# timmeinhardt/trackformer

Measured on AMD Instinct MI355X. Metric: frames/sec, TrackFormer-Deformable inference (ResNet-50, 1333x800, 300 object + 100 track queries, bs 1 per GPU); roofline = ms_deform_attn HBM GB/s, higher is better.
Workload: dtype f32 (dense layers as the fp16 split product on MFMA: two fp16 pieces per activation, three per weight scaled per output channel -- 22 + 1 significand bits per operand, the one dropped product < 2^-22 --, three terms, f32 accumulate)

## Files before the change

include/tf_fused.h:

```cpp
#ifndef TF_FUSED_H_
#define TF_FUSED_H_

#include <stdint.h>

#ifdef __cplusplus
extern "C" {
#endif

int tf_bias_act_f32(float *x, const float *bias, const float *residual, int64_t n, int C, int relu,
                    void *stream);

int tf_add_layernorm_f32(const float *x, const float *res, const float *gamma, const float *beta,
                         float *out, int64_t rows, int C, float eps, void *stream);

int tf_box_refine_f32(const float *delta, const float *ref, float *out, int64_t rows, int ref_dim, float eps, void *stream);

int tf_postprocess_pack_f32(const float *logits, const float *boxes, float *out, int64_t Q, int C, float img_h, float img_w,
                            int clip, void *stream);

int tf_groupnorm_nhwc_f32(const float *x, const float *gamma, const float *beta, float *out, double *workspace, int N,
                          int HW, int C, int G, float eps, int64_t x_image_stride, int64_t out_image_stride, void *stream);
int tf_groupnorm_stats_nhwc_f32(const float *x, double *workspace, int N, int HW, int C, int G, int64_t x_image_stride, void *stream);
int tf_groupnorm_relu_nhwc_f32(const float *x, const float *gamma, const float *beta, float *out, double *workspace, int N,
                               int HW, int C, int G, float eps, int64_t x_image_stride, int64_t out_image_stride, void *stream);
// ... 76 lines not shown
                         void *stream);

int tf_conv_packed_f32(const float *x, const void *w_packed, const float *bias, const float *residual, float *y, float *workspace,
                       int ksplit, int nimg, int hin, int win, int cin, int cout, int ks, int stride, int relu, int terms,
                       void *stream);

int tf_linear_res_ln_f32(const float *x, const void *w_packed, const float *bias, const float *residual, const float *ln_weight,
                         const float *ln_bias, float ln_eps, float *y, int64_t M, int K, int N, int terms, void *stream);

int tf_ffn_fused_f32(const float *x, const void *w1_packed, const float *b1, const void *w2_packed, const float *b2,
                     const float *residual, const float *ln_weight, const float *ln_bias, float ln_eps, float *y, int64_t M,
                     int d_model, int d_ffn, int terms, void *stream);

typedef struct tf_proj_group {
    const void *w_packed;
    const float *bias;
    float *y;
    int N;
    int add_x2;
} tf_proj_group;
int tf_linear_groups_f32(const float *x, const float *x2, const tf_proj_group *groups, int ngroups, int64_t M, int K, int terms,
                         void *stream);

int tf_mha_core_f32(const float *q, const float *k, const float *v, float *out, const unsigned char *key_mask,
                    int N, int Lq, int Lk, int H, int D, int ldq, int ldk, int ldv, int ldo, float scale,
                    void *stream);

int tf_nms_host_f32(const float *boxes, const float *scores, int n, float iou_threshold, int64_t *keep, int *n_keep);

#ifdef __cplusplus
}
#endif
#endif
```

include/tf_msda.h:

```cpp
#ifndef TF_MSDA_H_
#define TF_MSDA_H_

#include <stdint.h>

#ifdef __cplusplus
extern "C" {
#endif

#define TF_MSDA_ABI_VERSION 9
#define TF_MSDA_MAX_LEVELS 16

typedef enum tf_msda_status {
    TF_MSDA_OK = 0,
    TF_MSDA_ERR_NULL_POINTER = -1,
    TF_MSDA_ERR_BAD_DIMS = -2,
    TF_MSDA_ERR_SHAPE_SUM = -3,
    TF_MSDA_ERR_LAUNCH = -4,
    TF_MSDA_ERR_NO_DEVICE = -5,
    TF_MSDA_ERR_WORKSPACE = -6
} tf_msda_status;

int tf_msda_abi_version(void);

const char *tf_msda_strerror(int status);

int tf_msda_last_hip_error(void);

const char *tf_msda_last_kernel(void);

int tf_msda_set_tiled(int mode);

int tf_msda_set_option(const char *name, int value);
// ... 79 lines not shown
```

trackformer_amd/_cabi.py:

```python
import ctypes
import os

_PKG_DIR = os.path.dirname(os.path.abspath(__file__))
LIB_PATH = os.environ.get("TF_MSDA_LIB") or os.path.join(_PKG_DIR, "lib", "libtf_msda.so")

EXPORTED_SYMBOLS = (
    "tf_msda_abi_version",
    "tf_msda_strerror",
    "tf_msda_last_hip_error",
    "tf_msda_last_kernel",
    "tf_msda_set_tiled",
    "tf_msda_set_option",
    "tf_msda_debug_trace_buffer",
    "tf_msda_forward_fused_f32",
    "tf_msda_forward_f32",
    "tf_msda_forward_f64",
    "tf_msda_forward_f32_dshapes",
    "tf_msda_forward_f64_dshapes",
    "tf_msda_backward_f32",
    "tf_msda_backward_f64",
    "tf_msda_backward_f32_dshapes",
    "tf_msda_backward_f64_dshapes",
    "tf_msda_backward_det_workspace_bytes",
    "tf_msda_backward_det_f32",
# ... 26 lines not shown
    "tf_conv1x1_strided_split_f32",
    "tf_conv1x1_splitk_f32",
    "tf_linear_packed_bytes",
    "tf_linear_pack_weight_f32",
    "tf_linear_packed_f32",
    "tf_linear_grad_stats_workspace_bytes",
    "tf_linear_grad_stats_f32",
    "tf_linear_wgrad_workspace_bytes",
    "tf_linear_wgrad_split_f32",
    "tf_linear_dgrad_packed_f32",
    "tf_add_layernorm_train_f32",
    "tf_add_layernorm_bwd_workspace_bytes",
    "tf_add_layernorm_bwd_f32",
    "tf_set_criterion_fwd_f32",
    "tf_set_criterion_bwd_f32",
    "tf_match_cost_f32",
    "tf_mask_loss_workspace_bytes",
    "tf_mask_loss_fwd_f32",
    "tf_mask_loss_bwd_f32",
    "tf_linear_split_add_f32",
    "tf_ffn_fused_f32",
    "tf_linear_res_ln_f32",
    "tf_linear_groups_f32",
    "tf_conv_packed_f32",
    "tf_mha_core_f32",
    "tf_nms_host_f32",
)

ABI_VERSION = 9

_lib = None


class ProjGroup(ctypes.Structure):
    _fields_ = [("w_packed", ctypes.c_void_p), ("bias", ctypes.c_void_p), ("y", ctypes.c_void_p), ("N", ctypes.c_int),
                ("add_x2", ctypes.c_int)]


class MSDAError(RuntimeError):
    """Raised when libtf_msda.so reports a non-zero status."""


def lib():
    global _lib
    if _lib is not None:
        return _lib
    if not os.path.exists(LIB_PATH):
        raise RuntimeError(
            "trackformer_amd: native library %s not found. Build it with "
            "`python -m trackformer_amd.build` (needs hipcc); there is no CPU fallback." % LIB_PATH)
    import torch
    L = ctypes.CDLL(LIB_PATH)
# ... 67 lines not shown
        fn.argtypes = [vp, vp, vp, vp, vp, ci, ci, ci, ci, ctypes.c_float, ctypes.c_int64, ctypes.c_int64, vp]
    L.tf_linear_split_f32.restype = ci
    L.tf_linear_split_f32.argtypes = [vp, vp, vp, vp, vp, vp, vp, ctypes.c_int64, ci, ci, ci, vp]
    L.tf_linear_split_res_f32.restype = ci
    L.tf_linear_split_res_f32.argtypes = [vp, vp, vp, vp, vp, vp, vp, vp, ctypes.c_int64, ci, ci, ci, vp]
    L.tf_conv3x3_splitk_f32.restype = ci
    L.tf_conv3x3_splitk_f32.argtypes = [vp, vp, vp, vp, vp, vp, vp, vp, ci, ci, ci, ci, ci, ci, ci, ci, vp]
    L.tf_conv3x3_split_f32.restype = ci
    L.tf_conv3x3_split_f32.argtypes = [vp, vp, vp, vp, vp, vp, vp] + [ci] * 7 + [vp]
    L.tf_conv1x1_splitk_f32.restype = ci
    L.tf_conv1x1_splitk_f32.argtypes = [vp, vp, vp, vp, vp, vp, vp, vp, ci, ci, ci, ci, ci, ci, ci, ci, vp]
    L.tf_conv1x1_strided_split_f32.restype = ci
    L.tf_conv1x1_strided_split_f32.argtypes = [vp, vp, vp, vp, vp, vp, vp] + [ci] * 7 + [vp]
    L.tf_linear_packed_bytes.restype = ctypes.c_int64
    L.tf_linear_packed_bytes.argtypes = [ci, ci, ci]
    L.tf_linear_pack_weight_f32.restype = ci
    L.tf_linear_pack_weight_f32.argtypes = [vp, vp, ci, ci, ci, vp]
    L.tf_linear_res_ln_f32.restype = ci
    L.tf_linear_res_ln_f32.argtypes = [vp, vp, vp, vp, vp, vp, ctypes.c_float, vp, ctypes.c_int64, ci, ci, ci, vp]
    L.tf_ffn_fused_f32.restype = ci
    L.tf_ffn_fused_f32.argtypes = [vp, vp, vp, vp, vp, vp, vp, vp, ctypes.c_float, vp, ctypes.c_int64, ci, ci, ci, vp]
    L.tf_linear_groups_f32.restype = ci
    L.tf_linear_groups_f32.argtypes = [vp, vp, ctypes.POINTER(ProjGroup), ci, ctypes.c_int64, ci, ci, vp]
    L.tf_linear_split_add_f32.restype = ci
    L.tf_linear_split_add_f32.argtypes = [vp, vp, vp, vp, vp, vp, vp, vp, ctypes.c_int64, ci, ci, vp]
    L.tf_linear_packed_f32.restype = ci
    L.tf_linear_packed_f32.argtypes = [vp, vp, vp, vp, vp, ctypes.c_int64, ci, ci, ci, ci, vp]
    i64 = ctypes.c_int64
    L.tf_linear_grad_stats_workspace_bytes.restype = i64
    L.tf_linear_grad_stats_workspace_bytes.argtypes = [i64, ci, ci, ci]
    L.tf_linear_grad_stats_f32.restype = ci
    L.tf_linear_grad_stats_f32.argtypes = [vp, vp, vp, vp, i64, i64, ci, ci, ci, vp]
    L.tf_linear_wgrad_workspace_bytes.restype = i64
    L.tf_linear_wgrad_workspace_bytes.argtypes = [i64, ci, ci]
    L.tf_linear_wgrad_split_f32.restype = ci
    L.tf_linear_wgrad_split_f32.argtypes = [vp, vp, vp, vp, vp, vp, i64, i64, ci, ci, ci, vp]
    L.tf_linear_dgrad_packed_f32.restype = ci
    L.tf_linear_dgrad_packed_f32.argtypes = [vp, vp, vp, vp, i64, ci, ci, ci, vp]
    L.tf_add_layernorm_train_f32.restype = ci
    L.tf_add_layernorm_train_f32.argtypes = [vp, vp, vp, vp, vp, vp, i64, ci, ctypes.c_float, vp]
    L.tf_add_layernorm_bwd_workspace_bytes.restype = i64
    L.tf_add_layernorm_bwd_workspace_bytes.argtypes = [i64, ci]
    L.tf_add_layernorm_bwd_f32.restype = ci
    L.tf_add_layernorm_bwd_f32.argtypes = [vp] * 9 + [i64, i64, ci, vp]
    cf = ctypes.c_float
    L.tf_set_criterion_fwd_f32.restype = ci
# ... 29 lines not shown
```

trackformer_amd/backbone.py:

```python
from collections import OrderedDict
from typing import Dict, List

import torch
import torch.nn.functional as F
from torch import nn

from . import fused
from .nested import NestedTensor, all_valid_mask, is_all_valid
from .position_encoding import build_position_encoding


import os as _os

CHANNELS_LAST = _os.environ.get("TF_BACKBONE_NCHW", "0") != "1"


_conv1x1_split = _os.environ.get("TF_CONV1X1_SPLIT", "1") != "0"


_conv3x3_split = _os.environ.get("TF_CONV3X3_SPLIT", "1") != "0"


def _parse_skip(text):
    out = set()
# ... 259 lines not shown
            and maxpool.padding == 1 and maxpool.dilation == 1 and not maxpool.ceil_mode):
        return None
    b = cache.get(conv1, bn1)
    w = cache.weight
    y = None
    if (conv1.kernel_size == (7, 7) and conv1.stride == (2, 2) and conv1.padding == (3, 3) and conv1.dilation == (1, 1)
            and conv1.groups == 1):
        fuse_pool = fused.stem_pool_fused_enabled()
        y = fused.stem_conv(x, w, None if fuse_pool else b, relu=not fuse_pool)
        if y is not None and not fuse_pool:
            return maxpool(y)
    if y is None:
        if not fused.stem_pool_fused_enabled():
            return None
        y = F.conv2d(x, w, None, conv1.stride, conv1.padding, conv1.dilation, conv1.groups)
    pooled = fused.bias_relu_maxpool(y, b)
    if pooled is None:
        if fused.bias_act_(y, b, None, True) is None:
            y = F.relu_(y + b.reshape(1, -1, 1, 1))
        pooled = maxpool(y)
    return pooled


class Bottleneck(nn.Module):
    expansion = 4

    def __init__(self, inplanes, planes, stride=1, downsample=None, dilation=1,
                 norm_layer=FrozenBatchNorm2d):
        super().__init__()
        self.conv1 = nn.Conv2d(inplanes, planes, kernel_size=1, bias=False)
        self.bn1 = norm_layer(planes)
        self.conv2 = nn.Conv2d(planes, planes, kernel_size=3, stride=stride, padding=dilation,
                               dilation=dilation, bias=False)
        self.bn2 = norm_layer(planes)
        self.conv3 = nn.Conv2d(planes, planes * self.expansion, kernel_size=1, bias=False)
        self.bn3 = norm_layer(planes * self.expansion)
        self.relu = nn.ReLU(inplace=True)
        self.downsample = downsample
        self.stride = stride
        self._folds = [_FoldCache() for _ in range(4)]

    def forward(self, x):
        fold = _fold_mode(self, x)
        out = _conv_bn(x, self.conv1, self.bn1, self._folds[0], True, fold)
        out = _conv_bn(out, self.conv2, self.bn2, self._folds[1], True, fold)
        if self.downsample is not None:
            x = _conv_bn(x, self.downsample[0], self.downsample[1], self._folds[3], False, fold)
        return _conv_bn(out, self.conv3, self.bn3, self._folds[2], True, fold, residual=x)


class ResNet(nn.Module):

    def __init__(self, layers, num_classes=1000, replace_stride_with_dilation=None,
                 norm_layer=FrozenBatchNorm2d):
        super().__init__()
        if replace_stride_with_dilation is None:
            replace_stride_with_dilation = [False, False, False]
        if len(replace_stride_with_dilation) != 3:
            raise ValueError("replace_stride_with_dilation should be None or a 3-element tuple")
        self._norm_layer = norm_layer
        self.inplanes = 64
        self.dilation = 1
        self.conv1 = nn.Conv2d(3, 64, kernel_size=7, stride=2, padding=3, bias=False)
        self.bn1 = norm_layer(64)
        self.relu = nn.ReLU(inplace=True)
        self.maxpool = nn.MaxPool2d(kernel_size=3, stride=2, padding=1)
        self.layer1 = self._make_layer(64, layers[0])
        self.layer2 = self._make_layer(128, layers[1], 2, replace_stride_with_dilation[0])
        self.layer3 = self._make_layer(256, layers[2], 2, replace_stride_with_dilation[1])
        self.layer4 = self._make_layer(512, layers[3], 2, replace_stride_with_dilation[2])
        self.avgpool = nn.AdaptiveAvgPool2d((1, 1))
# ... 16 lines not shown
        if stride != 1 or self.inplanes != planes * Bottleneck.expansion:
            downsample = nn.Sequential(
                nn.Conv2d(self.inplanes, planes * Bottleneck.expansion, kernel_size=1, stride=stride,
                          bias=False),
                norm_layer(planes * Bottleneck.expansion))
        layers = [Bottleneck(self.inplanes, planes, stride, downsample, previous_dilation, norm_layer)]
        self.inplanes = planes * Bottleneck.expansion
        for _ in range(1, blocks):
            layers.append(Bottleneck(self.inplanes, planes, dilation=self.dilation,
                                     norm_layer=norm_layer))
        return nn.Sequential(*layers)

    def stem(self, x):
        fold = _fold_mode(self.conv1, x) if self.training else int(_inference_mode(self))
        if fold == 1:
            pooled = _stem_pooled(x, self.conv1, self.bn1, self.maxpool, self._stem_fold)
            if pooled is not None:
                return pooled
        x = _conv_bn(x, self.conv1, self.bn1, self._stem_fold, True, fold)
        return self.maxpool(x)

    def forward(self, x):
        x = self.stem(x)
        x = self.layer4(self.layer3(self.layer2(self.layer1(x))))
        return self.fc(torch.flatten(self.avgpool(x), 1))


_RESNET_DEPTHS = {"resnet50": [3, 4, 6, 3], "resnet101": [3, 4, 23, 3]}


def resnet(name: str, replace_stride_with_dilation=None, norm_layer=FrozenBatchNorm2d) -> ResNet:
    if name not in _RESNET_DEPTHS:
        raise ValueError("unsupported backbone %r (have %s)" % (name, sorted(_RESNET_DEPTHS)))
    return ResNet(_RESNET_DEPTHS[name], replace_stride_with_dilation=replace_stride_with_dilation,
                  norm_layer=norm_layer)


class IntermediateLayerGetter(nn.ModuleDict):

    def __init__(self, model: nn.Module, return_layers: Dict[str, str]):
        if not set(return_layers).issubset(name for name, _ in model.named_children()):
            raise ValueError("return_layers are not present in model")
        remaining = dict(return_layers)
        kept = OrderedDict()
        for name, module in model.named_children():
            kept[name] = module
            remaining.pop(name, None)
            if not remaining:
                break
        super().__init__(kept)
        self.return_layers = dict(return_layers)
        self._fold = _FoldCache()

    def forward(self, x):
        out = OrderedDict()
        fold = _fold_mode(self["conv1"], x) if (self.training and "conv1" in self) else int(_inference_mode(self))
        fused_stem = fold == 1 and all(k in self for k in ("conv1", "bn1", "relu"))
        pooled_stem = (fused_stem and "maxpool" in self
                       and not any(k in self.return_layers for k in ("conv1", "bn1", "relu", "maxpool")))
        skip = ()
        for name, module in self.items():
            if name in skip or (fused_stem and name in ("bn1", "relu")):
                continue
            if fused_stem and name == "conv1":
                pooled = _stem_pooled(x, self["conv1"], self["bn1"], self["maxpool"], self._fold) if pooled_stem else None
                if pooled is not None:
                    x, skip = pooled, ("maxpool",)
                    continue
                x = _conv_bn(x, self["conv1"], self["bn1"], self._fold, True, 1)
            else:
                x = module(x)
            if name in self.return_layers:
                out[self.return_layers[name]] = x
        return out


class BackboneBase(nn.Module):
    def __init__(self, backbone: nn.Module, train_backbone: bool, return_interm_layers: bool):
        super().__init__()
        for name, parameter in backbone.named_parameters():
            if not train_backbone or not any(k in name for k in ("layer2", "layer3", "layer4")):
                parameter.requires_grad_(False)
        if return_interm_layers:
            return_layers = {"layer1": "0", "layer2": "1", "layer3": "2", "layer4": "3"}
            self.strides = [4, 8, 16, 32]
# ... 58 lines not shown
```

trackformer_amd/build.py:

```python
import hashlib
import os
import shutil
import subprocess
import sys
from concurrent.futures import ThreadPoolExecutor

PKG_DIR = os.path.dirname(os.path.abspath(__file__))
REPO_DIR = os.path.dirname(PKG_DIR)
CSRC = os.path.join(PKG_DIR, "csrc")
LIB_DIR = os.path.join(PKG_DIR, "lib")
INCLUDE = os.path.join(REPO_DIR, "include")
GFX_ARCH = "gfx950"

_TARGETS = [
    ("libtf_msda.so", ["msda_hip.hip", "msda_pquad.hip", "fused_ops.hip", "linear_split.hip", "linear_stream.hip", "mha_core.hip", "ffn_fused.hip", "stem_conv.hip", "msda_host.cpp"], []),
]


def _hipcc():
    exe = shutil.which("hipcc") or "/opt/rocm/bin/hipcc"
    if not os.path.exists(exe):
        raise RuntimeError("hipcc not found (expected on PATH or at /opt/rocm/bin/hipcc)")
    return exe

# ... 37 lines not shown
        src_paths = [os.path.join(CSRC, s) for s in srcs]
        flags = ["--offload-arch=" + GFX_ARCH, "-O3", "-std=c++17", "-fPIC", "-I" + INCLUDE,
                 "-Wno-pass-failed"] + extra
        key = _key(src_paths + headers, flags)
        if not force and not _stale(out, key):
            continue
        obj_dir = os.path.join(LIB_DIR, "obj")
        os.makedirs(obj_dir, exist_ok=True)
        objs = [os.path.join(obj_dir, os.path.splitext(s)[0] + ".o") for s in srcs]
        with ThreadPoolExecutor(max_workers=len(srcs)) as pool:
            list(pool.map(lambda so: _run([_hipcc()] + flags + ["-c", so[0], "-o", so[1]], verbose),
                          zip(src_paths, objs)))
        _run([_hipcc(), "--offload-arch=" + GFX_ARCH, "-shared", "-fPIC", "-pthread"] + objs + ["-o", out], verbose)
        _stamp(out, key)
        built.append(out)
    built += _build_tools(force, verbose)
    return built


def _build_tools(force, verbose):
    out_dir = os.path.join(REPO_DIR, "tools", "bin")
    lib = os.path.join(LIB_DIR, "libtf_msda.so")
    built = []
    for name in ("msda_bench", "linear_bench", "ffn_bench", "proj_groups_bench"):
        src = os.path.join(REPO_DIR, "tools", name + ".cpp")
        if not os.path.exists(src):
            continue
        os.makedirs(out_dir, exist_ok=True)
        out = os.path.join(out_dir, name)
        flags = ["--offload-arch=" + GFX_ARCH, "-O2", "-std=c++17", "-I" + INCLUDE]
        headers = [os.path.join(INCLUDE, f) for f in os.listdir(INCLUDE) if f.endswith(".h")]
        key = _key([src] + headers, flags)
        if not force and not _stale(out, key) and os.path.getmtime(out) >= os.path.getmtime(lib):
            continue
        _run([_hipcc()] + flags + [src, "-L" + LIB_DIR, "-ltf_msda",
                                   "-Wl,-rpath,$ORIGIN/../../trackformer_amd/lib", "-o", out], verbose)
        _stamp(out, key)
        built.append(out)
    return built


if __name__ == "__main__":
    res = build_all(force="--force" in sys.argv, verbose=True)
    print("built:" if res else "up to date", *res)
```

trackformer_amd/csrc/ffn_fused.hip:

```cpp
#include <hip/hip_runtime.h>

#include <stdint.h>
#include <stdlib.h>

#include <type_traits>

#include "host_dispatch.h"
#include "msda_common.h"
#include "split_product.h"
#include "tf_fused.h"
#include "tf_msda.h"

namespace {

template <int D>
struct Geo {
    static_assert(D == 256 || D == 288, "hidden sizes of the reference's configurations");
    static constexpr int NW = D == 256 ? 4 : 3;
    static constexpr int NT = NW * 64;
    static constexpr int TJ = D / 32 / NW;
    static constexpr int XS = D + 8;
    static constexpr int CH = NW * 32;
    static constexpr int HS = CH + 8;
    static constexpr int KQ1 = D / 16;
// ... 653 lines not shown
        }
#pragma unroll 1
        for (int k = 0; k < pg.nchunk[ph][1]; ++k, ++ci) {
            const ChunkW nxt = chunk_of(pg.chunk[min(ci + 1, total - 1)]);
            run_chunk(std::true_type{}, cur, nxt, pg.chunk[ci]);
            cur = nxt;
        }
    }
}

template <int SP, int TI>
int launch_groups(const float *x, const float *x2, int M, const ProjGroups &pg, hipStream_t s)
{
    constexpr size_t tile = linln_lds_bytes<256>(TI, Split<SP>::NA), lds_max = tile + 2 * 4 * kMaxProjCols;
    static_assert(lds_max <= 160 * 1024, "the activation tile and the tables do not fit the LDS of a CU");
    const size_t lds = tile + 2 * 4 * (size_t)pg.ncols;
    const void *fn = (const void *)&linear_groups_kernel<SP, TI>;
    if (lds_max > 64 * 1024 && !tfm::raise_dynamic_lds_limit(fn)) return TF_MSDA_ERR_LAUNCH;
    const int blocks = (M + 32 * TI - 1) / (32 * TI);
    void *argv[] = {(void *)&x, (void *)&x2, (void *)&M, (void *)&pg};
    return hipLaunchKernel(fn, dim3((unsigned)blocks), dim3(256), argv, lds, s) == hipSuccess ? TF_MSDA_OK : TF_MSDA_ERR_LAUNCH;
}

}

extern "C" int tf_linear_groups_f32(const float *x, const float *x2, const tf_proj_group *groups, int ngroups, int64_t M, int K, int terms,
                                    void *stream)
{
    if (!x || !groups) return TF_MSDA_ERR_NULL_POINTER;
    if (ngroups < 1 || ngroups > kMaxProjGroups) return TF_MSDA_ERR_BAD_DIMS;
    for (int i = 0; i < ngroups; ++i)
        if (!groups[i].w_packed || !groups[i].y || (groups[i].add_x2 && !x2)) return TF_MSDA_ERR_NULL_POINTER;
    const int sp = split_scheme(terms);
    if (M <= 0 || K != 256 || sp == 0 || (M + 128) * (int64_t)K * 4 > 0xFFFFFFFFLL) return TF_MSDA_ERR_BAD_DIMS;
    uintptr_t al = reinterpret_cast<uintptr_t>(x) | reinterpret_cast<uintptr_t>(x2);
    ProjGroups pg{};
    for (int pass = 0; pass < 2; ++pass)
        for (int i = 0; i < ngroups; ++i) {
            const tf_proj_group &g = groups[i];
            if ((g.add_x2 != 0) != (pass == 1)) continue;
            if (g.N <= 0 || (g.N % 32) != 0 || (M + 128) * (int64_t)g.N * 4 > 0xFFFFFFFFLL) return TF_MSDA_ERR_BAD_DIMS;
            al |= reinterpret_cast<uintptr_t>(g.w_packed) | reinterpret_cast<uintptr_t>(g.bias) | reinterpret_cast<uintptr_t>(g.y);
            pg.g[pg.ng++] = ProjGroup{static_cast<const u32x4 *>(g.w_packed), g.bias, g.y, g.N, pg.ncols};
            pg.ncols += (g.N + 255) / 256 * 256;
            if (pass == 0) pg.nplain = pg.ng;
        }
// ... 59 lines not shown
```

trackformer_amd/csrc/host_dispatch.h:

```cpp
#ifndef TF_HOST_DISPATCH_H_
#define TF_HOST_DISPATCH_H_

#include <hip/hip_runtime.h>

#include <stdlib.h>

#include <atomic>
#include <mutex>

namespace tfm {

struct KernelVariant {
    const void *fn;
    const char *name;
};

inline bool env_flag(const char *name, bool dflt)
{
    const char *e = getenv(name);
    return e ? e[0] != '0' : dflt;
}

inline int num_cus()
{
// ... 25 lines not shown
inline bool raise_dynamic_lds_limit(const void *fn)
{
    static LdsLimitSlot slots[kLdsLimitSlots];
    static std::mutex mu;
    int dev = 0;
    if (hipGetDevice(&dev) != hipSuccess || dev < 0 || dev >= 64) return false;
    const unsigned long long bit = 1ull << dev;
    LdsLimitSlot *s = lds_limit_find(slots, fn);
    if (s && (s->devs.load(std::memory_order_acquire) & bit)) return true;
    std::lock_guard<std::mutex> guard(mu);
    s = lds_limit_find(slots, fn);
    if (s && (s->devs.load(std::memory_order_relaxed) & bit)) return true;
    if (hipFuncSetAttribute(fn, hipFuncAttributeMaxDynamicSharedMemorySize, 160 * 1024) != hipSuccess) return false;
    for (int i = 0; !s && i < kLdsLimitSlots; ++i)
        if (!slots[i].fn.load(std::memory_order_relaxed)) {
            s = &slots[i];
            s->fn.store(fn, std::memory_order_release);
        }
    if (s) s->devs.fetch_or(bit, std::memory_order_release);
    return true;
}

enum DenseKnob { kKnobFfnTi, kKnobFfnTailSplit, kKnobLinlnTi, kKnobGroupsTi, kKnobLinearStreamTi, kKnobConvHalo, kKnobLinearDma,
                 kKnobMhaMfma, kKnobWgradMsplit, kKnobCount };
int dense_knob(DenseKnob k);
int dense_knob_set(const char *name, int v, int unknown);

}

#endif
```

trackformer_amd/csrc/msda_hip.hip:

```cpp
#include <hip/hip_runtime.h>

#include <limits.h>
#include <stdint.h>
#include <stdio.h>
#include <stdlib.h>
#include <string.h>

#include <atomic>
#include <type_traits>

#include "tf_msda.h"
#include "msda_common.h"
#include "msda_dispatch.h"
#include "msda_quad_geom.h"

namespace {
using namespace tfm;

constexpr int kThreads = 256;
constexpr int kLdsChunkBudget = 48 * 1024;

constexpr int kLevelTableBytes = 3 * TF_MSDA_MAX_LEVELS * (int)sizeof(int);

template <typename T, int VEC>
// ... 1808 lines not shown
#include "msda_fused_bwd.h"

}

namespace tfm {
void note_kernel(const char *name) { g_last_kernel = name; }

struct DenseKnobDesc {
    const char *name, *env;
    int dflt;
    bool flag;
    int lo, hi, other;
};
constexpr DenseKnobDesc kDenseKnobs[kKnobCount] = {
    {"ffn_ti", "TF_FFN_TI", 3, false, 1, 3, 3},
    {"ffn_tail_split", "TF_FFN_TAIL_SPLIT", 1, true, 0, 1, 0},
    {"linln_ti", "TF_LINLN_TI", 0, false, 0, 3, 0},
    {"groups_ti", nullptr, 0, false, 1, 3, 0},
    {"linear_stream_ti", "TF_LINEAR_STREAM_TI", 0, false, 1, 4, 0},
    {"conv_halo", "TF_CONV_HALO", 1, true, 0, 1, 0},
    {"linear_dma", "TF_LINEAR_DMA", 0, false, 0, 9, 0},
    {"mha_mfma", "TF_MHA_MFMA", 1, false, 0, 2, 1},
    {"wgrad_msplit", nullptr, 0, false, 1, 64, 0},
};
static std::atomic<int> g_dense_knob[kKnobCount];

static int dense_knob_accept(const DenseKnobDesc &d, int v) { return d.flag ? v != 0 : (v >= d.lo && v <= d.hi ? v : d.other); }

int dense_knob(DenseKnob k)
{
    int cur = g_dense_knob[k].load(std::memory_order_relaxed);
    if (cur == 0) {
        const DenseKnobDesc &d = kDenseKnobs[k];
        int v = d.dflt;
        if (d.env && d.flag) v = env_flag(d.env, d.dflt != 0);
        else if (const char *e = d.env ? getenv(d.env) : nullptr) v = dense_knob_accept(d, atoi(e));
        if (g_dense_knob[k].compare_exchange_strong(cur, v + 1)) cur = v + 1;
    }
    return cur - 1;
}

int dense_knob_set(const char *name, int v, int unknown)
{
    for (int k = 0; k < kKnobCount; ++k)
        if (strcmp(name, kDenseKnobs[k].name) == 0) {
            const int prev = dense_knob((DenseKnob)k);
// ... 191 lines not shown
```

trackformer_amd/fused.py:

```python
import os
import threading

import torch
import torch.nn.functional as F

from . import _cabi


def _stream(device):
    return torch.cuda.current_stream(device).cuda_stream


def _param_ok(t, x):
    return (t.device == x.device and t.dtype == torch.float32 and t.is_contiguous()
            and t.data_ptr() % 16 == 0)


_weight_epoch = 0
_route_epoch = 0


def weight_epoch():
    return _weight_epoch

# ... 603 lines not shown
    if (a.data_ptr() | _ptr(b)) & 15:
        return None
    cols = 0
    for w, bias, _add in groups:
        if not (w.dtype == torch.float32 and w.dim() == 2 and w.is_contiguous() and w.device == x.device and w.shape[1] == K
                and w.shape[0] % 32 == 0 and (M + 128) * w.shape[0] * 4 <= 0xFFFFFFFF):
            return None
        if bias is not None and not (_param_ok(bias, x) and bias.numel() == w.shape[0]):
            return None
        cols += (w.shape[0] + 255) // 256 * 256
    if cols > 4096:
        return None
    packed = [_packed_weight(w, None) for w, _b, _add in groups]
    if any(p is None for p in packed):
        return None
    descs = (_cabi.ProjGroup * len(groups))()
    with torch.cuda.device(x.device):
        ys = [torch.empty((M, w.shape[0]), dtype=torch.float32, device=x.device) for w, _b, _add in groups]
        for d, (w, bias, add), p, y in zip(descs, groups, packed, ys):
            d.w_packed, d.bias, d.y, d.N, d.add_x2 = p.data_ptr(), (bias.data_ptr() if bias is not None else None), y.data_ptr(), w.shape[0], int(bool(add))
        rc = _cabi.lib().tf_linear_groups_f32(a.data_ptr(), _ptr(b) or None, descs, len(groups), M, K, _terms(), _stream(x.device))
    _cabi.check(rc, "tf_linear_groups_f32")
    return [y.view(*x.shape[:-1], y.shape[1]) for y in ys]


def conv3x3(x, w_taps, bias, relu, stride):
    if not (_split_linear and x.is_cuda and x.dtype == torch.float32 and x.dim() == 4
            and x.is_contiguous(memory_format=torch.channels_last) and w_taps.dtype == torch.float32
            and w_taps.dim() == 2 and w_taps.is_contiguous() and w_taps.device == x.device):
        return None
    n, cin, h, w = x.shape
    cout = w_taps.shape[0]
    ks = 3 if w_taps.shape[1] == 9 * cin else 1
    if w_taps.shape[1] != ks * ks * cin or cin % 32 or stride not in (1, 2) or x.numel() == 0:
        return None
    if bias is not None and not (bias.dtype == torch.float32 and bias.is_contiguous() and bias.numel() == cout
                                 and bias.device == x.device):
        return None
    pad = 1 if ks == 3 else 0
    ho, wo = (h + 2 * pad - ks) // stride + 1, (w + 2 * pad - ks) // stride + 1
    cin_ok = cin % 64 == 0 or (ks == 3 and stride == 1 and _conv_halo and cin % 32 == 0)
    stream_route = (_conv_stream and _conv_stream_wins(n * ho * wo, cout) and cin_ok and not (x.data_ptr() & 15)
                    and n * h * w * cin * 4 < 0xC0000000 and (n * ho * wo + 256) * cout * 4 < 0xC0000000)
    halo = ks == 3 and stride == 1 and _conv_halo and stream_route
    ksplit = _conv_ksplit(n * ho * wo, ks * ks * cin, cout, _HALO_KSPLIT_POLICY if halo else None)
    if ks == 1 and (ksplit < _CONV1X1_MIN_PIECES or not _conv1x1_splitk):
# ... 730 lines not shown
```

Baseline: 375.5.

## Fuse bottleneck conv3 with next block's conv1 in one 1x1 pair kernel

Adds a HIP kernel that computes a bottleneck's conv3 (with bias, residual add and ReLU) and, from the same tile held in LDS, the next block's conv1 (with bias and ReLU). The ResNet layer runner now threads the precomputed conv1 output into the next block. This avoids re-reading the wide conv3 output from HBM and saves one kernel launch per pair. It is routed only for selected layer1/layer3 shapes with enough rows. The cost is a larger LDS footprint, more complex weight streaming, and extra Python routing logic.

```diff
diff --git a/include/tf_fused.h b/include/tf_fused.h
--- a/include/tf_fused.h
+++ b/include/tf_fused.h
@@ -122,6 +122,9 @@
 int tf_linear_groups_f32(const float *x, const float *x2, const tf_proj_group *groups, int ngroups, int64_t M, int K, int terms,
                          void *stream);
 
+int tf_conv1x1_pair_f32(const float *x, const void *w3_packed, const float *bias3, const float *residual, float *y,
+                        const void *w1_packed, const float *bias1, float *h, int64_t M, int K, int N, int N2, int terms, void *stream);
+
 int tf_mha_core_f32(const float *q, const float *k, const float *v, float *out, const unsigned char *key_mask,
                     int N, int Lq, int Lk, int H, int D, int ldq, int ldk, int ldv, int ldo, float scale,
                     void *stream);
diff --git a/include/tf_msda.h b/include/tf_msda.h
--- a/include/tf_msda.h
+++ b/include/tf_msda.h
@@ -7,7 +7,7 @@
 extern "C" {
 #endif
 
-#define TF_MSDA_ABI_VERSION 9
+#define TF_MSDA_ABI_VERSION 10
 #define TF_MSDA_MAX_LEVELS 16
 
 typedef enum tf_msda_status {
diff --git a/trackformer_amd/_cabi.py b/trackformer_amd/_cabi.py
--- a/trackformer_amd/_cabi.py
+++ b/trackformer_amd/_cabi.py
@@ -72,12 +72,13 @@
     "tf_ffn_fused_f32",
     "tf_linear_res_ln_f32",
     "tf_linear_groups_f32",
+    "tf_conv1x1_pair_f32",
     "tf_conv_packed_f32",
     "tf_mha_core_f32",
     "tf_nms_host_f32",
 )
 
-ABI_VERSION = 9
+ABI_VERSION = 10
 
 _lib = None
 
@@ -191,6 +192,8 @@
     L.tf_ffn_fused_f32.argtypes = [vp, vp, vp, vp, vp, vp, vp, vp, ctypes.c_float, vp, ctypes.c_int64, ci, ci, ci, vp]
     L.tf_linear_groups_f32.restype = ci
     L.tf_linear_groups_f32.argtypes = [vp, vp, ctypes.POINTER(ProjGroup), ci, ctypes.c_int64, ci, ci, vp]
+    L.tf_conv1x1_pair_f32.restype = ci
+    L.tf_conv1x1_pair_f32.argtypes = [vp, vp, vp, vp, vp, vp, vp, vp, ctypes.c_int64, ci, ci, ci, ci, vp]
     L.tf_linear_split_add_f32.restype = ci
     L.tf_linear_split_add_f32.argtypes = [vp, vp, vp, vp, vp, vp, vp, vp, ctypes.c_int64, ci, ci, vp]
     L.tf_linear_packed_f32.restype = ci
diff --git a/trackformer_amd/backbone.py b/trackformer_amd/backbone.py
--- a/trackformer_amd/backbone.py
+++ b/trackformer_amd/backbone.py
@@ -305,6 +305,60 @@
     return pooled
 
 
+def _pair_conv_ok(conv, bn):
+    return (isinstance(bn, FrozenBatchNorm2d) and conv.kernel_size == (1, 1) and conv.stride == (1, 1) and conv.padding == (0, 0)
+            and conv.groups == 1 and not conv.training and _split_route_allowed(conv))
+
+
+def _bottleneck_pair(out, identity, block, nxt, fold):
+    if not (fold == 1 and fused.bottleneck_pair_enabled() and _conv1x1_split and CHANNELS_LAST and out.is_cuda
+            and isinstance(nxt, Bottleneck) and _pair_conv_ok(block.conv3, block.bn3) and _pair_conv_ok(nxt.conv1, nxt.bn1)
+            and nxt.conv1.in_channels == block.conv3.out_channels
+            and fused.bottleneck_pair_routed(block.conv3.in_channels, block.conv3.out_channels, nxt.conv1.out_channels,
+                                             out.shape[0] * out.shape[2] * out.shape[3])):
+        return None
+    n, cin, h, w = out.shape
+    cout = block.conv3.out_channels
+    if not (out.dtype == torch.float32 and out.is_contiguous(memory_format=torch.channels_last) and identity.shape == (n, cout, h, w)
+            and identity.dtype == torch.float32 and identity.is_contiguous(memory_format=torch.channels_last)):
+        return None
+    if _fold_mode(nxt, identity) != 1:
+        return None
+    b3 = block._folds[2].get(block.conv3, block.bn3)
+    b1 = nxt._folds[0].get(nxt.conv1, nxt.bn1)
+    w3, w1 = block._folds[2].weight2d, nxt._folds[0].weight2d
+    if w3 is None or w1 is None:
+        return None
+    res = fused.conv1x1_pair(out.permute(0, 2, 3, 1).reshape(n * h * w, cin), w3, b3,
+                             identity.permute(0, 2, 3, 1).reshape(n * h * w, cout), w1, b1)
+    if res is None:
+        return None
+    y2, h2 = res
+    return y2.view(n, h, w, cout).permute(0, 3, 1, 2), h2.view(n, h, w, h2.shape[1]).permute(0, 3, 1, 2)
+
+
+def _run_layers(layers, x):
+    blocks = [list(layer) for layer in layers]
+    if not (fused.bottleneck_pair_enabled() and x.is_cuda and not torch.is_grad_enabled()
+            and all(isinstance(layer, nn.Sequential) and bl and all(isinstance(b, Bottleneck) and not b.training for b in bl)
+                    for layer, bl in zip(layers, blocks))):
+        outs = []
+        for layer in layers:
+            x = layer(x)
+            outs.append(x)
+        return outs
+    outs, head = [], None
+    for li, bl in enumerate(blocks):
+        for bi, b in enumerate(bl):
+            nxt = bl[bi + 1] if bi + 1 < len(bl) else (blocks[li + 1][0] if li + 1 < len(blocks) else None)
+            if nxt is None:
+                x = b(x, head=head)
+            else:
+                x, head = b(x, head=head, nxt=nxt)
+        outs.append(x)
+    return outs
+
+
 class Bottleneck(nn.Module):
     expansion = 4
 
@@ -323,13 +377,16 @@
         self.stride = stride
         self._folds = [_FoldCache() for _ in range(4)]
 
-    def forward(self, x):
+    def forward(self, x, head=None, nxt=None):
         fold = _fold_mode(self, x)
-        out = _conv_bn(x, self.conv1, self.bn1, self._folds[0], True, fold)
+        out = head if head is not None else _conv_bn(x, self.conv1, self.bn1, self._folds[0], True, fold)
         out = _conv_bn(out, self.conv2, self.bn2, self._folds[1], True, fold)
         if self.downsample is not None:
             x = _conv_bn(x, self.downsample[0], self.downsample[1], self._folds[3], False, fold)
-        return _conv_bn(out, self.conv3, self.bn3, self._folds[2], True, fold, residual=x)
+        if nxt is None:
+            return _conv_bn(out, self.conv3, self.bn3, self._folds[2], True, fold, residual=x)
+        pair = _bottleneck_pair(out, x, self, nxt, fold)
+        return pair if pair is not None else (_conv_bn(out, self.conv3, self.bn3, self._folds[2], True, fold, residual=x), None)
 
 
 class ResNet(nn.Module):
@@ -392,7 +449,7 @@
 
     def forward(self, x):
         x = self.stem(x)
-        x = self.layer4(self.layer3(self.layer2(self.layer1(x))))
+        x = _run_layers([self.layer1, self.layer2, self.layer3, self.layer4], x)[-1]
         return self.fc(torch.flatten(self.avgpool(x), 1))
 
 
@@ -429,8 +486,20 @@
         pooled_stem = (fused_stem and "maxpool" in self
                        and not any(k in self.return_layers for k in ("conv1", "bn1", "relu", "maxpool")))
         skip = ()
+        names = list(self.keys())
         for name, module in self.items():
             if name in skip or (fused_stem and name in ("bn1", "relu")):
+                continue
+            if name == "layer1" and isinstance(module, nn.Sequential):
+                run = []
+                for n in names[names.index(name):]:
+                    if not (n.startswith("layer") and isinstance(self[n], nn.Sequential)):
+                        break
+                    run.append(n)
+                for n, x in zip(run, _run_layers([self[n] for n in run], x)):
+                    if n in self.return_layers:
+                        out[self.return_layers[n]] = x
+                skip = tuple(run)
                 continue
             if fused_stem and name == "conv1":
                 pooled = _stem_pooled(x, self["conv1"], self["bn1"], self["maxpool"], self._fold) if pooled_stem else None
diff --git a/trackformer_amd/build.py b/trackformer_amd/build.py
--- a/trackformer_amd/build.py
+++ b/trackformer_amd/build.py
@@ -83,7 +83,7 @@
     out_dir = os.path.join(REPO_DIR, "tools", "bin")
     lib = os.path.join(LIB_DIR, "libtf_msda.so")
     built = []
-    for name in ("msda_bench", "linear_bench", "ffn_bench", "proj_groups_bench"):
+    for name in ("msda_bench", "linear_bench", "ffn_bench", "proj_groups_bench", "bottleneck_pair_bench"):
         src = os.path.join(REPO_DIR, "tools", name + ".cpp")
         if not os.path.exists(src):
             continue
diff --git a/trackformer_amd/csrc/conv1x1_pair.h b/trackformer_amd/csrc/conv1x1_pair.h
--- /dev/null
+++ b/trackformer_amd/csrc/conv1x1_pair.h
@@ -0,0 +1,271 @@
+#ifndef TF_CONV1X1_PAIR_H_
+#define TF_CONV1X1_PAIR_H_
+
+constexpr int kPairMaxN = 1024;
+
+template <int SP, int K, int N2, int TI>
+struct PairGeo {
+    static_assert((K == 64 || K == 128 || K == 256) && (N2 == 64 || N2 == 128 || N2 == 256) && (TI == 1 || TI == 2), "shapes of ResNet's layers 1-3");
+    static constexpr int BM = 32 * TI, XS = K + 8, CH = 128, HS = CH + 8;
+    static constexpr int KQ1 = K / 16, U1 = KQ1 / 2;
+    static constexpr int T2 = N2 / 32, WJ = T2 < 4 ? T2 : 4, WI = 4 / WJ, TJ2 = T2 / WJ;
+    static constexpr int TI2 = TI >= WI ? TI / WI : 1;
+    static constexpr int U2 = (CH / 16) * TJ2 / 2;
+    static constexpr int UPC = U1 + U2;
+    static constexpr int RING = UPC % 4 == 0 ? 4 : (Split<SP>::NB == 3 ? 3 : 6);
+    static constexpr int AHEAD = RING - 2;
+    static_assert(UPC % RING == 0 && AHEAD >= 1 && AHEAD < UPC, "geometry");
+    static constexpr size_t tiles_bytes = (size_t)Split<SP>::NA * BM * (XS + HS) * 2;
+};
+constexpr size_t pair_lds_budget = 80 * 1024;
+template <int SP, int K>
+constexpr bool pair_has_64_rows() { return PairGeo<SP, K, 64, 2>::tiles_bytes + 2 * 4 * kPairMaxN <= pair_lds_budget; }
+
+template <int SP, int K, int N2, int TI>
+__global__ void __launch_bounds__(256, 2)
+conv1x1_pair_kernel(const float *__restrict__ X, const u32x4 *__restrict__ W3p, const float *__restrict__ b3, const float *__restrict__ R,
+                    float *__restrict__ Y, const u32x4 *__restrict__ W1p, const float *__restrict__ b1, float *__restrict__ H, int M, int N)
+{
+    using G = PairGeo<SP, K, N2, TI>;
+    constexpr int BM = G::BM, XS = G::XS, HS = G::HS, KQ1 = G::KQ1, U1 = G::U1, U2 = G::U2, UPC = G::UPC, RING = G::RING;
+    constexpr int TJ2 = G::TJ2, TI2 = G::TI2, WJ = G::WJ;
+    constexpr int NA = Split<SP>::NA, NB = Split<SP>::NB, US = 2 * NB;
+    constexpr bool F16 = Split<SP>::F16;
+    extern __shared__ __attribute__((aligned(16))) unsigned short s_f[];
+    unsigned short *const sX = s_f;
+    unsigned short *const sH = s_f + NA * BM * XS;
+    float *const sB3 = reinterpret_cast<float *>(s_f + NA * BM * (XS + HS));
+    float *const sR3 = sB3 + N;
+    const int tid = threadIdx.x, lane = tid & 63;
+    const int wave = __builtin_amdgcn_readfirstlane(tid >> 6);
+    const int m0 = blockIdx.x * BM;
+    const int nchunks = N >> 7, KQ2 = N >> 4;
+    const int wj = wave % WJ, wi = wave / WJ;
+    const bool owner2 = wi * TI2 < TI;
+    const int rt2 = owner2 ? wi * TI2 : 0;
+    const int frow = lane & 31, fk = (lane >> 5) * 8, c4l = 4 * (lane >> 5);
+
+    u32x4 ring[RING][US];
+    auto load_unit = [&](int c, auto uc, u32x4 (&dst)[US]) {
+        constexpr int u = decltype(uc)::value;
+        if constexpr (u < U1) {
+            const u32x4 *base = W3p + ((size_t)(c * 4 + wave) * KQ1 * NB + u * 2 * NB) * 64 + lane;
+#pragma unroll
+            for (int i = 0; i < US; ++i) dst[i] = base[i * 64];
+        } else if constexpr (TJ2 == 2) {
+            const int q = c * 8 + (u - U1);
+#pragma unroll
+            for (int j = 0; j < 2; ++j)
+#pragma unroll
+                for (int p = 0; p < NB; ++p) dst[j * NB + p] = W1p[(((size_t)(2 * wj + j) * KQ2 + q) * NB + p) * 64 + lane];
+        } else {
+            const u32x4 *base = W1p + (((size_t)wj * KQ2 + c * 8 + 2 * (u - U1)) * NB) * 64 + lane;
+#pragma unroll
+            for (int i = 0; i < US; ++i) dst[i] = base[i * 64];
+        }
+    };
+    static_for<G::AHEAD>([&](auto uc) { load_unit(0, uc, ring[decltype(uc)::value]); });
+    __builtin_amdgcn_sched_barrier(0);
+
+    const __amdgpu_buffer_rsrc_t xrs = __builtin_amdgcn_make_buffer_rsrc(const_cast<float *>(X), 0, (unsigned)((size_t)M * K * 4), 0x00020000);
+    const unsigned ybytes = (unsigned)((size_t)M * N * 4);
+    const __amdgpu_buffer_rsrc_t rrs = __builtin_amdgcn_make_buffer_rsrc(const_cast<float *>(R), 0, ybytes, 0x00020000);
+    const __amdgpu_buffer_rsrc_t yrs = __builtin_amdgcn_make_buffer_rsrc(Y, 0, ybytes, 0x00020000);
+    const __amdgpu_buffer_rsrc_t hrs = __builtin_amdgcn_make_buffer_rsrc(H, 0, (unsigned)((size_t)M * N2 * 4), 0x00020000);
+    const __amdgpu_buffer_rsrc_t b3rs = __builtin_amdgcn_make_buffer_rsrc(const_cast<float *>(b3 ? b3 : X), 0, b3 ? (unsigned)N * 4u : 0u, 0x00020000);
+    const __amdgpu_buffer_rsrc_t b1rs = __builtin_amdgcn_make_buffer_rsrc(const_cast<float *>(b1 ? b1 : X), 0, b1 ? (unsigned)N2 * 4u : 0u, 0x00020000);
+    const float *const r3 = reinterpret_cast<const float *>(W3p + (size_t)((N + 255) / 256 * 8) * KQ1 * NB * 64);
+    const float *const r1 = reinterpret_cast<const float *>(W1p + (size_t)((N2 + 255) / 256 * 8) * KQ2 * NB * 64);
+
+    f32x4 rv[TI][4];
+    const unsigned yoff = (unsigned)((m0 + frow) * N + wave * 32 + c4l) * 4u;
+    auto load_res = [&](int c) {
+#pragma unroll
+        for (int i = 0; i < TI; ++i)
+#pragma unroll
+            for (int g = 0; g < 4; ++g)
+                rv[i][g] = __builtin_bit_cast(f32x4, __builtin_amdgcn_raw_buffer_load_b128(rrs, yoff + (unsigned)(i * 32 * N + c * 128 + 8 * g) * 4u, 0, 0));
+    };
+    load_res(0);
+    for (int c = tid * 4; c < N; c += 4 * 256) {
+        *reinterpret_cast<f32x4 *>(sB3 + c) = __builtin_bit_cast(f32x4, __builtin_amdgcn_raw_buffer_load_b128(b3rs, (unsigned)c * 4u, 0, 0));
+        if constexpr (F16) *reinterpret_cast<f32x4 *>(sR3 + c) = *reinterpret_cast<const f32x4 *>(r3 + c);
+    }
+    {
+        constexpr int C4 = K / 4, NV = BM * C4 / 256;
+        static_assert(BM * C4 % 256 == 0, "tile does not divide among the threads");
+        f32x4 xr[NV];
+#pragma unroll
+        for (int it = 0; it < NV; ++it) {
+            const int idx = it * 256 + tid, row = idx / C4, c4 = idx - row * C4;
+            xr[it] = __builtin_bit_cast(f32x4, __builtin_amdgcn_raw_buffer_load_b128(xrs, (unsigned)((m0 + row) * K + c4 * 4) * 4u, 0, 0));
+        }
+        __builtin_amdgcn_sched_barrier(0);
+#pragma unroll
+        for (int it = 0; it < NV; ++it) {
+            const int idx = it * 256 + tid, row = idx / C4, c4 = idx - row * C4;
+            u32x2 pc[NA];
+            split4<SP>(xr[it], pc);
+#pragma unroll
+            for (int p = 0; p < NA; ++p) *reinterpret_cast<u32x2 *>(&sX[(p * BM + row) * XS + c4 * 4]) = pc[p];
+        }
+    }
+    __syncthreads();
+
+    f32x16 acc2[TI2][TJ2];
+#pragma unroll
+    for (int i = 0; i < TI2; ++i)
+#pragma unroll
+        for (int j = 0; j < TJ2; ++j)
+#pragma unroll
+            for (int e = 0; e < 16; ++e) acc2[i][j][e] = 0.f;
+    const int xoff = frow * XS + fk, hoff = (rt2 * 32 + frow) * HS + fk;
+
+    for (int c = 0; c < nchunks; ++c) {
+        const int cn = min(c + 1, nchunks - 1);
+        auto prefetch = [&](auto uc) {
+            constexpr int ahead = decltype(uc)::value + G::AHEAD;
+            if constexpr (ahead < UPC) load_unit(c, std::integral_constant<int, ahead>{}, ring[ahead % RING]);
+            else load_unit(cn, std::integral_constant<int, ahead - UPC>{}, ring[ahead % RING]);
+        };
+        f32x16 acc1[TI][1];
+#pragma unroll
+        for (int i = 0; i < TI; ++i)
+#pragma unroll
+            for (int e = 0; e < 16; ++e) acc1[i][0][e] = 0.f;
+        u32x4 xf[2][TI][NA];
+        auto read_x = [&](auto stc) {
+            constexpr int st = decltype(stc)::value;
+#pragma unroll
+            for (int i = 0; i < TI; ++i)
+#pragma unroll
+                for (int p = 0; p < NA; ++p)
+                    xf[st & 1][i][p] = *reinterpret_cast<const u32x4 *>(&sX[(p * BM + i * 32) * XS + xoff + st * 16]);
+        };
+        read_x(std::integral_constant<int, 0>{});
+        static_for<KQ1>([&](auto stc) {
+            constexpr int st = decltype(stc)::value;
+            if constexpr ((st & 1) == 0) prefetch(std::integral_constant<int, st / 2>{});
+            if constexpr (st + 1 < KQ1) read_x(std::integral_constant<int, st + 1>{});
+            __builtin_amdgcn_sched_barrier(0);
+            const u32x4 (&cur)[US] = ring[(st / 2) % RING];
+            u32x4 wf[1][NB];
+#pragma unroll
+            for (int p = 0; p < NB; ++p) wf[0][p] = cur[(st & 1) * NB + p];
+            mfma_tiles<SP, TI, 1, false>(acc1, xf[st & 1], wf);
+        });
+
+        __syncthreads();
+        const int ccol = c * 128 + wave * 32 + c4l;
+#pragma unroll
+        for (int g = 0; g < 4; ++g) {
+            const f32x4 bv = *reinterpret_cast<const f32x4 *>(sB3 + ccol + 8 * g);
+            f32x4 sv = {1.f, 1.f, 1.f, 1.f};
+            if constexpr (F16) sv = *reinterpret_cast<const f32x4 *>(sR3 + ccol + 8 * g);
+#pragma unroll
+            for (int i = 0; i < TI; ++i) {
+                f32x4 yv;
+#pragma unroll
+                for (int e = 0; e < 4; ++e) {
+                    float t = F16 ? __builtin_fmaf(acc1[i][0][4 * g + e], sv[e], bv[e]) : acc1[i][0][4 * g + e] + bv[e];
+                    t += rv[i][g][e];
+                    yv[e] = t < 0.f ? 0.f : t;
+                }
+                __builtin_amdgcn_raw_buffer_store_b128(__builtin_bit_cast(u32x4, yv), yrs, yoff + (unsigned)(i * 32 * N + c * 128 + 8 * g) * 4u, 0,
+                                                       tfm::kStoreAux);
+                u32x2 pc[NA];
+                split4<SP>(yv, pc);
+                const int o = (i * 32 + frow) * HS + wave * 32 + 8 * g + c4l;
+#pragma unroll
+                for (int p = 0; p < NA; ++p) *reinterpret_cast<u32x2 *>(&sH[p * BM * HS + o]) = pc[p];
+            }
+        }
+        if (c + 1 < nchunks) load_res(c + 1);
+        __syncthreads();
+
+        u32x4 hf[2][TI2][NA];
+        auto read_h = [&](auto vc) {
+            constexpr int kv = decltype(vc)::value;
+#pragma unroll
+            for (int i = 0; i < TI2; ++i)
+#pragma unroll
+                for (int p = 0; p < NA; ++p)
+                    hf[kv & 1][i][p] = *reinterpret_cast<const u32x4 *>(&sH[(p * BM + i * 32) * HS + hoff + kv * 16]);
+        };
+        read_h(std::integral_constant<int, 0>{});
+        static_for<G::CH / 16>([&](auto vc) {
+            constexpr int kv = decltype(vc)::value;
+            constexpr int u = U1 + (TJ2 == 2 ? kv : kv / 2);
+            if constexpr (TJ2 == 2 || (kv & 1) == 0) prefetch(std::integral_constant<int, u>{});
+            if constexpr (kv + 1 < G::CH / 16) read_h(std::integral_constant<int, kv + 1>{});
+            __builtin_amdgcn_sched_barrier(0);
+            const u32x4 (&cur)[US] = ring[u % RING];
+            u32x4 wf[TJ2][NB];
+#pragma unroll
+            for (int j = 0; j < TJ2; ++j)
+#pragma unroll
+                for (int p = 0; p < NB; ++p) wf[j][p] = cur[(TJ2 == 2 ? j : (kv & 1)) * NB + p];
+            mfma_tiles<SP, TI2, TJ2, false>(acc2, hf[kv & 1], wf);
+        });
+    }
+
+    if (owner2) {
+#pragma unroll
+        for (int j = 0; j < TJ2; ++j)
+#pragma unroll
+            for (int g = 0; g < 4; ++g) {
+                const int col = (TJ2 * wj + j) * 32 + 8 * g + c4l;
+                const f32x4 bv = __builtin_bit_cast(f32x4, __builtin_amdgcn_raw_buffer_load_b128(b1rs, (unsigned)col * 4u, 0, 0));
+                f32x4 sv = {1.f, 1.f, 1.f, 1.f};
+                if constexpr (F16) sv = *reinterpret_cast<const f32x4 *>(r1 + col);
+#pragma unroll
+                for (int i = 0; i < TI2; ++i) {
+                    f32x4 hv;
+#pragma unroll
+                    for (int e = 0; e < 4; ++e) {
+                        const float t = F16 ? __builtin_fmaf(acc2[i][j][4 * g + e], sv[e], bv[e]) : acc2[i][j][4 * g + e] + bv[e];
+                        hv[e] = t < 0.f ? 0.f : t;
+                    }
+                    __builtin_amdgcn_raw_buffer_store_b128(__builtin_bit_cast(u32x4, hv), hrs,
+                                                           (unsigned)((m0 + (rt2 + i) * 32 + frow) * N2 + col) * 4u, 0, tfm::kStoreAux);
+                }
+            }
+    }
+}
+
+template <int SP, int K, int N2, int TI>
+int launch_pair(const float *x, const u32x4 *w3, const float *b3, const float *res, float *y, const u32x4 *w1, const float *b1, float *h,
+                int M, int N, hipStream_t s)
+{
+    using G = PairGeo<SP, K, N2, TI>;
+    static_assert(G::tiles_bytes + 2 * 4 * kPairMaxN <= 160 * 1024, "the two tiles and the tables do not fit the LDS of a CU");
+    const size_t lds = G::tiles_bytes + 2 * 4 * (size_t)N;
+    const void *fn = (const void *)&conv1x1_pair_kernel<SP, K, N2, TI>;
+    if (G::tiles_bytes + 2 * 4 * kPairMaxN > 64 * 1024 && !tfm::raise_dynamic_lds_limit(fn)) return TF_MSDA_ERR_LAUNCH;
+    const int blocks = (M + G::BM - 1) / G::BM;
+    void *argv[] = {(void *)&x, (void *)&w3, (void *)&b3, (void *)&res, (void *)&y, (void *)&w1, (void *)&b1, (void *)&h, (void *)&M, (void *)&N};
+    return hipLaunchKernel(fn, dim3((unsigned)blocks), dim3(256), argv, lds, s) == hipSuccess ? TF_MSDA_OK : TF_MSDA_ERR_LAUNCH;
+}
+
+template <int SP, int K, int N2>
+int dispatch_pair(const float *x, const u32x4 *w3, const float *b3, const float *res, float *y, const u32x4 *w1, const float *b1, float *h,
+                  int M, int N, hipStream_t s)
+{
+    if constexpr (pair_has_64_rows<SP, K>())
+        if (tfm::dense_knob(tfm::kKnobPairTi) != 1) return launch_pair<SP, K, N2, 2>(x, w3, b3, res, y, w1, b1, h, M, N, s);
+    return launch_pair<SP, K, N2, 1>(x, w3, b3, res, y, w1, b1, h, M, N, s);
+}
+
+template <int SP>
+int dispatch_pair_shape(int K, int N2, const float *x, const u32x4 *w3, const float *b3, const float *res, float *y, const u32x4 *w1,
+                        const float *b1, float *h, int M, int N, hipStream_t s)
+{
+    if (K == 64 && N2 == 64) return dispatch_pair<SP, 64, 64>(x, w3, b3, res, y, w1, b1, h, M, N, s);
+    if (K == 64 && N2 == 128) return dispatch_pair<SP, 64, 128>(x, w3, b3, res, y, w1, b1, h, M, N, s);
+    if (K == 128 && N2 == 128) return dispatch_pair<SP, 128, 128>(x, w3, b3, res, y, w1, b1, h, M, N, s);
+    if (K == 128 && N2 == 256) return dispatch_pair<SP, 128, 256>(x, w3, b3, res, y, w1, b1, h, M, N, s);
+    if (K == 256 && N2 == 256) return dispatch_pair<SP, 256, 256>(x, w3, b3, res, y, w1, b1, h, M, N, s);
+    return TF_MSDA_ERR_BAD_DIMS;
+}
+
+#endif
diff --git a/trackformer_amd/csrc/ffn_fused.hip b/trackformer_amd/csrc/ffn_fused.hip
--- a/trackformer_amd/csrc/ffn_fused.hip
+++ b/trackformer_amd/csrc/ffn_fused.hip
@@ -699,6 +699,28 @@
     return hipLaunchKernel(fn, dim3((unsigned)blocks), dim3(256), argv, lds, s) == hipSuccess ? TF_MSDA_OK : TF_MSDA_ERR_LAUNCH;
 }
 
+#include "conv1x1_pair.h"
+
+}
+
+extern "C" int tf_conv1x1_pair_f32(const float *x, const void *w3_packed, const float *bias3, const float *residual, float *y,
+                                   const void *w1_packed, const float *bias1, float *h, int64_t M, int K, int N, int N2, int terms,
+                                   void *stream)
+{
+    if (!x || !w3_packed || !residual || !y || !w1_packed || !h) return TF_MSDA_ERR_NULL_POINTER;
+    const int sp = split_scheme(terms);
+    if (M <= 0 || K <= 0 || N <= 0 || N2 <= 0 || sp == 0) return TF_MSDA_ERR_BAD_DIMS;
+    if ((K % 32) != 0 || (N % 128) != 0 || N > kPairMaxN || (N2 % 32) != 0) return TF_MSDA_ERR_BAD_DIMS;
+    const int64_t widest = N > K ? (N > N2 ? N : N2) : (K > N2 ? K : N2);
+    if ((M + 64) * widest * 4 >= 0xC0000000LL) return TF_MSDA_ERR_BAD_DIMS;
+    uintptr_t al = reinterpret_cast<uintptr_t>(x) | reinterpret_cast<uintptr_t>(w3_packed) | reinterpret_cast<uintptr_t>(bias3) |
+                   reinterpret_cast<uintptr_t>(residual) | reinterpret_cast<uintptr_t>(y) | reinterpret_cast<uintptr_t>(w1_packed) |
+                   reinterpret_cast<uintptr_t>(bias1) | reinterpret_cast<uintptr_t>(h);
+    if (al & 15) return TF_MSDA_ERR_BAD_DIMS;
+    const u32x4 *w3 = static_cast<const u32x4 *>(w3_packed), *w1 = static_cast<const u32x4 *>(w1_packed);
+    hipStream_t s = static_cast<hipStream_t>(stream);
+    return sp == 3 ? dispatch_pair_shape<3>(K, N2, x, w3, bias3, residual, y, w1, bias1, h, (int)M, N, s)
+                   : dispatch_pair_shape<16>(K, N2, x, w3, bias3, residual, y, w1, bias1, h, (int)M, N, s);
 }
 
 extern "C" int tf_linear_groups_f32(const float *x, const float *x2, const tf_proj_group *groups, int ngroups, int64_t M, int K, int terms,
diff --git a/trackformer_amd/csrc/host_dispatch.h b/trackformer_amd/csrc/host_dispatch.h
--- a/trackformer_amd/csrc/host_dispatch.h
+++ b/trackformer_amd/csrc/host_dispatch.h
@@ -71,7 +71,7 @@
 }
 
 enum DenseKnob { kKnobFfnTi, kKnobFfnTailSplit, kKnobLinlnTi, kKnobGroupsTi, kKnobLinearStreamTi, kKnobConvHalo, kKnobLinearDma,
-                 kKnobMhaMfma, kKnobWgradMsplit, kKnobCount };
+                 kKnobMhaMfma, kKnobWgradMsplit, kKnobPairTi, kKnobCount };
 int dense_knob(DenseKnob k);
 int dense_knob_set(const char *name, int v, int unknown);
 
diff --git a/trackformer_amd/csrc/msda_hip.hip b/trackformer_amd/csrc/msda_hip.hip
--- a/trackformer_amd/csrc/msda_hip.hip
+++ b/trackformer_amd/csrc/msda_hip.hip
@@ -1854,6 +1854,7 @@
     {"linear_dma", "TF_LINEAR_DMA", 0, false, 0, 9, 0},
     {"mha_mfma", "TF_MHA_MFMA", 1, false, 0, 2, 1},
     {"wgrad_msplit", nullptr, 0, false, 1, 64, 0},
+    {"pair_ti", nullptr, 2, false, 1, 2, 2},
 };
 static std::atomic<int> g_dense_knob[kKnobCount];
 
diff --git a/trackformer_amd/fused.py b/trackformer_amd/fused.py
--- a/trackformer_amd/fused.py
+++ b/trackformer_amd/fused.py
@@ -649,6 +649,94 @@
         rc = _cabi.lib().tf_linear_groups_f32(a.data_ptr(), _ptr(b) or None, descs, len(groups), M, K, _terms(), _stream(x.device))
     _cabi.check(rc, "tf_linear_groups_f32")
     return [y.view(*x.shape[:-1], y.shape[1]) for y in ys]
+
+
+_BOTTLENECK_PAIR_ROUTED = {
+    (64, 256, 64): True,
+    (64, 256, 128): False,
+    (128, 512, 128): False,
+    (128, 512, 256): False,
+    (256, 1024, 256): True,
+}
+
+
+def _parse_bottleneck_pair(v):
+    v = str(v).strip().lower()
+    if v in ("", "0", "off", "false"):
+        return False
+    return "all" if v == "all" else True
+
+
+_bottleneck_pair = _parse_bottleneck_pair(os.environ.get("TF_BOTTLENECK_PAIR", "1"))
+_BOTTLENECK_PAIR_MIN_ROWS = int(os.environ.get("TF_BOTTLENECK_PAIR_MIN_ROWS", "4096"))
+_bottleneck_pair_counts = {"pair": 0}
+
+
+def bottleneck_pair_enabled():
+    return _bottleneck_pair
+
+
+def set_bottleneck_pair(on):
+    global _bottleneck_pair
+    prev, _bottleneck_pair = _bottleneck_pair, _parse_bottleneck_pair("1" if on is True else on)
+    return _switched(prev, _bottleneck_pair)
+
+
+def bottleneck_pair_counts(reset=False):
+    out = dict(_bottleneck_pair_counts)
+    if reset:
+        _bottleneck_pair_counts["pair"] = 0
+    return out
+
+
+def set_bottleneck_pair_min_rows(n):
+    global _BOTTLENECK_PAIR_MIN_ROWS
+    prev, _BOTTLENECK_PAIR_MIN_ROWS = _BOTTLENECK_PAIR_MIN_ROWS, int(n)
+    return _switched(prev, _BOTTLENECK_PAIR_MIN_ROWS)
+
+
+def bottleneck_pair_routed(K, N, N2, M):
+    if not _bottleneck_pair:
+        return False
+    if _bottleneck_pair == "all":
+        return (K, N, N2) in _BOTTLENECK_PAIR_ROUTED
+    return M >= _BOTTLENECK_PAIR_MIN_ROWS and _BOTTLENECK_PAIR_ROUTED.get((K, N, N2), False)
+
+
+def conv1x1_pair(x, weight3, bias3, residual, weight1, bias1):
+    if not (_bottleneck_pair and _split_linear and x.is_cuda and x.dtype == torch.float32 and x.dim() == 2 and x.is_contiguous()
+            and x.numel()):
+        return None
+    if _split_terms == 16 and (_n_six_term_routes or debug_checks_active()):
+        return None
+    for w in (weight3, weight1):
+        if not (w.dtype == torch.float32 and w.dim() == 2 and w.is_contiguous() and w.device == x.device):
+            return None
+    M, K = x.shape
+    N, N2 = weight3.shape[0], weight1.shape[0]
+    if weight3.shape[1] != K or weight1.shape[1] != N or not bottleneck_pair_routed(K, N, N2, M):
+        return None
+    if not (residual is not None and residual.dtype == torch.float32 and residual.is_contiguous() and residual.device == x.device
+            and residual.shape == (M, N)):
+        return None
+    for b, n in ((bias3, N), (bias1, N2)):
+        if b is not None and not (_param_ok(b, x) and b.numel() == n):
+            return None
+    if (x.data_ptr() | residual.data_ptr()) & 15 or (M + 64) * max(K, N, N2) * 4 >= 0xC0000000:
+        return None
+    p3, p1 = _packed_weight(weight3, None), _packed_weight(weight1, None)
+    if p3 is None or p1 is None:
+        return None
+    with torch.cuda.device(x.device):
+        y = torch.empty((M, N), dtype=torch.float32, device=x.device)
+        h = torch.empty((M, N2), dtype=torch.float32, device=x.device)
+        rc = _cabi.lib().tf_conv1x1_pair_f32(x.data_ptr(), p3.data_ptr(), _ptr(bias3), residual.data_ptr(), y.data_ptr(), p1.data_ptr(),
+                                             _ptr(bias1), h.data_ptr(), M, K, N, N2, _terms(), _stream(x.device))
+    if rc == -2:
+        return None
+    _cabi.check(rc, "tf_conv1x1_pair_f32")
+    _bottleneck_pair_counts["pair"] += 1
+    return y, h
 
 
 def conv3x3(x, w_taps, bias, relu, stride):
```

Result: no change. 371.9 (-1.0%).
